# datawhalechina/torch-rechub

Measured on AMD Instinct MI355X. Metric: CTR train samples/sec, DeepFM Criteo-shape synthetic, higher is better.
Workload: dtype f32

## Files before the change

torch_rechub_amd/csrc/optim.hip:

```cpp
#include "common.h"
#include "wgrad_body.h"

namespace {

constexpr int kMaxTensors = 128;
constexpr int kMaxRing = 1024;
int g_sweep_grid = 0;
int g_deferred_grid = 512;
int g_gate_ns = 32000;
int g_stagger_ns = 15000;

constexpr int kVecPerThread = 4;
constexpr int kChunk4 = RH_BLOCK * kVecPerThread;

struct AdamArgs {
  const int64_t* tdesc;
  const double* hyper;
  int T;
  int zero_grad;
  int64_t total_vblocks;
  int64_t vb_prefix[kMaxTensors + 1];
};

__global__ void adam_prepare_kernel(double* hyper, int64_t* step, float* ring, int64_t ring_mask) {
  RH_CHAIN_PRIO();
  if (threadIdx.x == 0 && blockIdx.x == 0) {
    const int64_t t = *step + 1;
    *step = t;
    const double lr = hyper[0], b1 = hyper[1], b2 = hyper[2];
    const double bc1 = 1.0 - pow(b1, (double)t);
    const double bc2 = 1.0 - pow(b2, (double)t);
    hyper[8] = lr / bc1;
    hyper[9] = sqrt(bc2);
    hyper[10] = 1.0 - b1;
    hyper[11] = 1.0 - b2;
    hyper[12] = (double)t;
    const double A = hyper[8] * hyper[9], E = hyper[3] * hyper[9];
    hyper[13] = A;
    hyper[14] = E;
    if (ring != nullptr) {
      ring[2 * (t & ring_mask) + 0] = (float)A;
      ring[2 * (t & ring_mask) + 1] = (float)E;
    }
  }
}

struct AdamScalars {
  float b1, b2, wd, one_m_b1, one_m_b2;
  float c1wd, c2wd2;
  float A, E;
};

static __device__ __forceinline__ void adam_elem(float& p, float g, float& m, float& v, const AdamScalars& h, float A,
                                                 float E) {
  g = fmaf(h.wd, p, g);
  m = fmaf(h.one_m_b1, g - m, m);
  v = fmaf(h.one_m_b2, g * g, v * h.b2);
  p = fmaf(-A, m * __builtin_amdgcn_rcpf(__builtin_amdgcn_sqrtf(v) + E), p);
}
typedef float rh_v2f __attribute__((ext_vector_type(2)));
static __device__ __forceinline__ void adam_pair(rh_v2f& p, rh_v2f g, rh_v2f& m, rh_v2f& v, const AdamScalars& h,
                                                 float A, float E) {
  g = __builtin_elementwise_fma(rh_v2f{h.wd, h.wd}, p, g);
  m = __builtin_elementwise_fma(rh_v2f{h.one_m_b1, h.one_m_b1}, g - m, m);
  v = __builtin_elementwise_fma(rh_v2f{h.one_m_b2, h.one_m_b2}, g * g, v * h.b2);
  rh_v2f d = rh_v2f{__builtin_amdgcn_sqrtf(v.x), __builtin_amdgcn_sqrtf(v.y)} + E;
  d = rh_v2f{__builtin_amdgcn_rcpf(d.x), __builtin_amdgcn_rcpf(d.y)};
  p = __builtin_elementwise_fma(rh_v2f{-A, -A}, m * d, p);
}
static __device__ __forceinline__ void adam_pair_zero_g(rh_v2f& p, rh_v2f& m, rh_v2f& v, const AdamScalars& h, float A,
                                                        float E) {
  m = __builtin_elementwise_fma(rh_v2f{h.c1wd, h.c1wd}, p, m * h.b1);
  v = __builtin_elementwise_fma(rh_v2f{h.c2wd2, h.c2wd2}, p * p, v * h.b2);
  rh_v2f d = rh_v2f{__builtin_amdgcn_sqrtf(v.x), __builtin_amdgcn_sqrtf(v.y)} + E;
  d = rh_v2f{__builtin_amdgcn_rcpf(d.x), __builtin_amdgcn_rcpf(d.y)};
  p = __builtin_elementwise_fma(rh_v2f{-A, -A}, m * d, p);
}
static __device__ __forceinline__ void adam_f4_zero_g(float4& P, float4& M, float4& V, const AdamScalars& h, float A,
                                                      float E) {
  rh_v2f p0{P.x, P.y}, p1{P.z, P.w}, m0{M.x, M.y}, m1{M.z, M.w}, v0{V.x, V.y}, v1{V.z, V.w};
  adam_pair_zero_g(p0, m0, v0, h, A, E);
  adam_pair_zero_g(p1, m1, v1, h, A, E);
  P = make_float4(p0.x, p0.y, p1.x, p1.y);
  M = make_float4(m0.x, m0.y, m1.x, m1.y);
  V = make_float4(v0.x, v0.y, v1.x, v1.y);
}
static __device__ __forceinline__ void adam_f4(float4& P, const float4 G, float4& M, float4& V, const AdamScalars& h,
                                               float A, float E) {
  float4 Pz = P, Mz = M, Vz = V;
  adam_f4_zero_g(Pz, Mz, Vz, h, A, E);
  rh_v2f p0{P.x, P.y}, p1{P.z, P.w}, m0{M.x, M.y}, m1{M.z, M.w}, v0{V.x, V.y}, v1{V.z, V.w};
  adam_pair(p0, rh_v2f{G.x, G.y}, m0, v0, h, A, E);
  adam_pair(p1, rh_v2f{G.z, G.w}, m1, v1, h, A, E);
  P = make_float4(G.x == 0.f ? Pz.x : p0.x, G.y == 0.f ? Pz.y : p0.y, G.z == 0.f ? Pz.z : p1.x, G.w == 0.f ? Pz.w : p1.y);
  M = make_float4(G.x == 0.f ? Mz.x : m0.x, G.y == 0.f ? Mz.y : m0.y, G.z == 0.f ? Mz.z : m1.x, G.w == 0.f ? Mz.w : m1.y);
  V = make_float4(G.x == 0.f ? Vz.x : v0.x, G.y == 0.f ? Vz.y : v0.y, G.z == 0.f ? Vz.z : v1.x, G.w == 0.f ? Vz.w : v1.y);
}
static __device__ __forceinline__ AdamScalars load_scalars(const double* hyper) {
  AdamScalars h;
  h.b1 = (float)hyper[1];
  h.b2 = (float)hyper[2];
  h.wd = (float)hyper[4];
  h.one_m_b1 = (float)hyper[10];
  h.one_m_b2 = (float)hyper[11];
  h.c1wd = h.one_m_b1 * h.wd;
  h.c2wd2 = h.one_m_b2 * h.wd * h.wd;
  h.A = (float)hyper[13];
  h.E = (float)hyper[14];
  return h;
}

__global__ __launch_bounds__(RH_BLOCK) void adam_dense_kernel(const AdamArgs a) {
  const AdamScalars h = load_scalars(a.hyper);
  const int T = a.T;
  for (int64_t vb = blockIdx.x; vb < a.total_vblocks; vb += gridDim.x) {
    int lo = 0, hi = T;
    while (hi - lo > 1) {
      const int mid = (lo + hi) >> 1;
      if (a.vb_prefix[mid] <= vb) lo = mid; else hi = mid;
    }
    const int t = lo;
    float* p = reinterpret_cast<float*>(a.tdesc[0 * T + t]);
    float* g = reinterpret_cast<float*>(a.tdesc[1 * T + t]);
    float* m = reinterpret_cast<float*>(a.tdesc[2 * T + t]);
    float* v = reinterpret_cast<float*>(a.tdesc[3 * T + t]);
    const int64_t n4 = a.tdesc[4 * T + t] / 4;
    const int64_t base4 = (vb - a.vb_prefix[t]) * kChunk4;
    float4 P[kVecPerThread], Gv[kVecPerThread], M[kVecPerThread], V[kVecPerThread];
    bool ok[kVecPerThread];
#pragma unroll
    for (int k = 0; k < kVecPerThread; ++k) {
      const int64_t i4 = base4 + (int64_t)k * RH_BLOCK + threadIdx.x;
      ok[k] = i4 < n4;
      const int64_t j4 = ok[k] ? i4 : 0;
      P[k] = gload<float4>(p + j4 * 4);
      Gv[k] = gload<float4>(g + j4 * 4);
      M[k] = gload<float4>(m + j4 * 4);
      V[k] = gload<float4>(v + j4 * 4);
    }
#pragma unroll
    for (int k = 0; k < kVecPerThread; ++k) {
      if (!ok[k]) continue;
      const int64_t i4 = base4 + (int64_t)k * RH_BLOCK + threadIdx.x;
      const bool gnz = Gv[k].x != 0.f || Gv[k].y != 0.f || Gv[k].z != 0.f || Gv[k].w != 0.f;
      adam_f4(P[k], Gv[k], M[k], V[k], h, h.A, h.E);
      gstore<float4>(p + i4 * 4, P[k]);
      gstore<float4>(m + i4 * 4, M[k]);
      gstore<float4>(v + i4 * 4, V[k]);
      if (a.zero_grad && gnz) gstore<float4>(g + i4 * 4, f4_zero());
    }
  }
}


struct LazyTouchedArgs {
  const int64_t* ldesc;
  const int64_t* field_table;
  const int64_t* idesc;
  const double* hyper;
  const float* ring;
  int ring_mask;
  int T, B, F, spb;
  int* err;
  const int64_t* perm;
  const int64_t* pos;
  int64_t N;
  const int64_t* src_sparse;
  int Fd;
  const float* src_dense;
  int ND;
  const float* src_label;
  int64_t* sparse_out;
  float* dense_out;
  float* label_out;
  int look;
  int look_n;
  int64_t off;
};

struct LazySweepArgs {
  const int64_t* ldesc;
  const double* hyper;
  const float* ring;
  int ring_mask;
  int T;
  int flush;
  int64_t t_value;
  int64_t total_vblocks;
  int64_t vb_prefix[kMaxTensors + 1];
  int touch_blocks, touch_chunks, touch_period;
  int touch_i32;
  LazyTouchedArgs touch;
};

template <int LPR, typename IdxT, bool REFRESH, bool ASSEMBLE = false, bool LOOK = false, bool GRAD = !REFRESH>
static __device__ __forceinline__ void lazy_touched_body(const LazyTouchedArgs& a, int bx, int f);

template <int LPR, bool MERGED>
static __device__ __forceinline__ void lazy_sweep_body(const LazySweepArgs& a, const int bx_, const int gdim_) {
  constexpr int RPB = RH_BLOCK / LPR;
  constexpr int D = 4 * LPR;
  int64_t bid = bx_, nblk = gdim_;
  if (MERGED) {
    const int bx = bx_, P = a.touch_period;
    const int slot_ = bx / P;
    if (bx % P == 0 && slot_ < a.touch_blocks) {
      if (a.touch_i32)
        lazy_touched_body<LPR, int, false>(a.touch, slot_ % a.touch_chunks, slot_ / a.touch_chunks);
      else
        lazy_touched_body<LPR, int64_t, false>(a.touch, slot_ % a.touch_chunks, slot_ / a.touch_chunks);
      return;
    }
    bid = bx - (slot_ + 1 < a.touch_blocks ? slot_ + 1 : a.touch_blocks);
    nblk = (int64_t)gdim_ - a.touch_blocks;
  }
  AdamScalars h = load_scalars(a.hyper);
  const int t = a.t_value >= 0 ? (int)a.t_value : (int)a.hyper[12];
  if (a.t_value >= 0) {
    h.A = a.ring[2 * (t & a.ring_mask)];
    h.E = a.ring[2 * (t & a.ring_mask) + 1];
  }
  const int T = a.T;
  const int q = threadIdx.x % LPR;
  const int slot = threadIdx.x / LPR;
  __shared__ float ring_s[2 * kMaxRing];
  for (int i = threadIdx.x; i < 2 * (a.ring_mask + 1); i += RH_BLOCK) ring_s[i] = a.ring[i];
  __syncthreads();

  struct Unit {
    float *p, *g, *m, *v;
    int* last;
    int64_t r;
    int old;
    bool live, with_g, claimed;
    float4 P, M, V, G;
  };
  auto fetch = [&](int64_t vb, Unit& u) {
    u.live = false;
    if (vb >= a.total_vblocks) return;
    int lo = 0, hi = T;
    while (hi - lo > 1) {
      const int mid = (lo + hi) >> 1;
      if (a.vb_prefix[mid] <= vb) lo = mid; else hi = mid;
    }
    const int ti = lo;
    u.p = reinterpret_cast<float*>(a.ldesc[0 * T + ti]);
    u.g = reinterpret_cast<float*>(a.ldesc[1 * T + ti]);
    u.m = reinterpret_cast<float*>(a.ldesc[2 * T + ti]);
    u.v = reinterpret_cast<float*>(a.ldesc[3 * T + ti]);
    u.last = reinterpret_cast<int*>(a.ldesc[4 * T + ti]);
    const int64_t rows = a.ldesc[5 * T + ti];
    const int64_t K = a.ldesc[6 * T + ti];
    const int64_t w = a.flush ? rows : a.ldesc[7 * T + ti];
    const int64_t wstart = a.flush ? 0 : ((int64_t)(t - 1) % K) * w;
    const int64_t local = (vb - a.vb_prefix[ti]) * RPB + slot;
    u.r = wstart + local;
    if (local >= w || u.r >= rows) return;
    u.with_g = (K == 1);
    const bool claim = MERGED && K != 1;
    u.claimed = claim;
    if (claim) {
      u.old = t;
      if (q == 0) u.old = atomicMax(u.last + u.r, t);
      u.with_g = true;
    } else {
      u.old = gload<int>(u.last + u.r);
    }
    u.P = gload<float4>(u.p + u.r * D + q * 4);
    u.M = gload<float4>(u.m + u.r * D + q * 4);
    u.V = gload<float4>(u.v + u.r * D + q * 4);
    u.G = u.with_g ? gload<float4>(u.g + u.r * D + q * 4) : f4_zero();
    if (claim) u.old = __shfl(u.old, (int)(threadIdx.x % RH_WAVE) - q, RH_WAVE);
    u.live = true;
  };
  auto process = [&](Unit& u) {
    const bool work = u.live && u.old < t;
    const int first = work ? u.old + 1 : t;
    int j = wave_min_uniform(first);
    while (j < t) {
      const int nxt = wave_min_uniform(first > j ? first : t);
      if (first <= j) {
        int jj = j;
        for (; jj + 2 <= nxt; jj += 2) {
          const float2 ae0 = *reinterpret_cast<const float2*>(ring_s + 2 * (jj & a.ring_mask));
          const float2 ae1 = *reinterpret_cast<const float2*>(ring_s + 2 * ((jj + 1) & a.ring_mask));
          __builtin_amdgcn_sched_barrier(0);
          adam_f4_zero_g(u.P, u.M, u.V, h, ae0.x, ae0.y);
          adam_f4_zero_g(u.P, u.M, u.V, h, ae1.x, ae1.y);
        }
        if (jj < nxt) {
          const float2 ae = *reinterpret_cast<const float2*>(ring_s + 2 * (jj & a.ring_mask));
          adam_f4_zero_g(u.P, u.M, u.V, h, ae.x, ae.y);
        }
      }
      j = nxt;
    }
    if (work) {
      if (u.with_g) adam_f4(u.P, u.G, u.M, u.V, h, h.A, h.E);
      else adam_f4_zero_g(u.P, u.M, u.V, h, h.A, h.E);
      gstore<float4>(u.p + u.r * D + q * 4, u.P);
      gstore<float4>(u.m + u.r * D + q * 4, u.M);
      gstore<float4>(u.v + u.r * D + q * 4, u.V);
      if (u.with_g && (u.G.x != 0.f || u.G.y != 0.f || u.G.z != 0.f || u.G.w != 0.f))
        gstore<float4>(u.g + u.r * D + q * 4, f4_zero());
      if (q == 0 && !(MERGED && u.with_g && u.claimed)) u.last[u.r] = t;
    }
  };
  Unit ua, ub;
  fetch(bid, ua);
  for (int64_t vb = bid; vb < a.total_vblocks; vb += 2 * nblk) {
    fetch(vb + nblk, ub);
    process(ua);
    fetch(vb + 2 * nblk, ua);
    process(ub);
  }
}

template <int LPR, bool MERGED = false>
__global__ __launch_bounds__(RH_BLOCK) void adam_lazy_sweep_kernel(const LazySweepArgs a) {
  lazy_sweep_body<LPR, MERGED>(a, (int)blockIdx.x, (int)gridDim.x);
}

template <int LPR, int VPL>
static __device__ __forceinline__ void lazy_sweep_wide_body(const LazySweepArgs& a, const int bx_, const int gdim_) {
  constexpr int RPB = RH_BLOCK / LPR;
  constexpr int D = 4 * LPR * VPL;
  const int64_t bid = bx_, nblk = gdim_;
  AdamScalars h = load_scalars(a.hyper);
  const int t = (int)a.t_value;
  h.A = a.ring[2 * (t & a.ring_mask)];
  h.E = a.ring[2 * (t & a.ring_mask) + 1];
  const int T = a.T;
  const int q = threadIdx.x % LPR;
  const int slot = threadIdx.x / LPR;
  __shared__ float ring_s[2 * kMaxRing];
  for (int i = threadIdx.x; i < 2 * (a.ring_mask + 1); i += RH_BLOCK) ring_s[i] = a.ring[i];
  __syncthreads();
  struct Unit {
    float *p, *m, *v;
    int* last;
    int64_t off;
    int64_t r;
    int old;
    bool live;
    float4 P[VPL], M[VPL], V[VPL];
  };
  auto fetch = [&](int64_t vb, Unit& u) {
    u.live = false;
    if (vb >= a.total_vblocks) return;
    int lo = 0, hi = T;
    while (hi - lo > 1) {
      const int mid = (lo + hi) >> 1;
      if (a.vb_prefix[mid] <= vb) lo = mid; else hi = mid;
    }
    const int ti = lo;
    u.p = reinterpret_cast<float*>(a.ldesc[0 * T + ti]);
    u.m = reinterpret_cast<float*>(a.ldesc[2 * T + ti]);
    u.v = reinterpret_cast<float*>(a.ldesc[3 * T + ti]);
    u.last = reinterpret_cast<int*>(a.ldesc[4 * T + ti]);
    const int64_t rows = a.ldesc[5 * T + ti];
    const int64_t K = a.ldesc[6 * T + ti];
    const int64_t w = a.ldesc[7 * T + ti];
    const int64_t wstart = ((int64_t)(t - 1) % K) * w;
    const int64_t local = (vb - a.vb_prefix[ti]) * RPB + slot;
    u.r = wstart + local;
    if (local >= w || u.r >= rows) return;
    u.off = u.r * D + (int64_t)q * (4 * VPL);
    u.old = gload<int>(u.last + u.r);
#pragma unroll
    for (int k = 0; k < VPL; ++k) {
      u.P[k] = gload<float4>(u.p + u.off + 4 * k);
      u.M[k] = gload<float4>(u.m + u.off + 4 * k);
      u.V[k] = gload<float4>(u.v + u.off + 4 * k);
    }
    u.live = true;
  };
  auto process = [&](Unit& u) {
    const bool work = u.live && u.old < t;
    const int first = work ? u.old + 1 : t;
    int j = wave_min_uniform(first);
    while (j < t) {
      const int nxt = wave_min_uniform(first > j ? first : t);
      if (first <= j) {
        int jj = j;
        for (; jj + 2 <= nxt; jj += 2) {
          const float2 ae0 = *reinterpret_cast<const float2*>(ring_s + 2 * (jj & a.ring_mask));
          const float2 ae1 = *reinterpret_cast<const float2*>(ring_s + 2 * ((jj + 1) & a.ring_mask));
          __builtin_amdgcn_sched_barrier(0);
#pragma unroll
          for (int k = 0; k < VPL; ++k) adam_f4_zero_g(u.P[k], u.M[k], u.V[k], h, ae0.x, ae0.y);
#pragma unroll
          for (int k = 0; k < VPL; ++k) adam_f4_zero_g(u.P[k], u.M[k], u.V[k], h, ae1.x, ae1.y);
        }
        if (jj < nxt) {
          const float2 ae = *reinterpret_cast<const float2*>(ring_s + 2 * (jj & a.ring_mask));
#pragma unroll
          for (int k = 0; k < VPL; ++k) adam_f4_zero_g(u.P[k], u.M[k], u.V[k], h, ae.x, ae.y);
        }
      }
      j = nxt;
    }
    if (work) {
#pragma unroll
      for (int k = 0; k < VPL; ++k) {
        adam_f4_zero_g(u.P[k], u.M[k], u.V[k], h, h.A, h.E);
        gstore<float4>(u.p + u.off + 4 * k, u.P[k]);
        gstore<float4>(u.m + u.off + 4 * k, u.M[k]);
        gstore<float4>(u.v + u.off + 4 * k, u.V[k]);
      }
      if (q == 0) u.last[u.r] = t;
    }
  };
  Unit ua, ub;
  fetch(bid, ua);
  for (int64_t vb = bid; vb < a.total_vblocks; vb += 2 * nblk) {
    fetch(vb + nblk, ub);
    process(ua);
    fetch(vb + 2 * nblk, ua);
    process(ub);
  }
}

template <int LPR, int VPL>
__global__ __launch_bounds__(RH_BLOCK) void adam_lazy_sweep_wide_kernel(const LazySweepArgs a) {
  lazy_sweep_wide_body<LPR, VPL>(a, (int)blockIdx.x, (int)gridDim.x);
}

__global__ void stream_delay_kernel(const long long ticks) {
  const long long t0 = wall_clock64();
  while (wall_clock64() - t0 < ticks) __builtin_amdgcn_s_sleep(16);
}

__global__ void stream_gate_kernel(const long long* gate, const long long expected, const long long ticks, const long long timeout,
                                   int* err, long long* done_host, const long long done_value) {
  if (done_host != nullptr) __hip_atomic_store(done_host, done_value, __ATOMIC_RELAXED, __HIP_MEMORY_SCOPE_SYSTEM);
  const long long t0 = wall_clock64();
  while (__hip_atomic_load(gate, __ATOMIC_ACQUIRE, __HIP_MEMORY_SCOPE_AGENT) - expected < 0) {
    __builtin_amdgcn_s_sleep(8);
    if (wall_clock64() - t0 > timeout) {
      if (err != nullptr) atomicOr(err, RH_ERR_GATE_TIMEOUT);
      return;
    }
  }
  const int slot = 4 + 2 * (int)(expected & 3);
  const long long base = __hip_atomic_load(gate + slot, __ATOMIC_RELAXED, __HIP_MEMORY_SCOPE_AGENT);
  const long long opened = __hip_atomic_load(gate + slot + 1, __ATOMIC_RELAXED, __HIP_MEMORY_SCOPE_AGENT);
  while (__hip_atomic_load(gate + 2, __ATOMIC_RELAXED, __HIP_MEMORY_SCOPE_AGENT) - base < 1 && wall_clock64() - opened < ticks)
    __builtin_amdgcn_s_sleep(4);
}

static __device__ __forceinline__ void gate_open(long long* gate) {
  const long long idx = __hip_atomic_load(gate, __ATOMIC_RELAXED, __HIP_MEMORY_SCOPE_AGENT) + 1;
  const int slot = 4 + 2 * (int)(idx & 3);
  const long long now = (long long)wall_clock64();
  __hip_atomic_store(gate + slot, __hip_atomic_load(gate + 2, __ATOMIC_RELAXED, __HIP_MEMORY_SCOPE_AGENT), __ATOMIC_RELAXED,
                     __HIP_MEMORY_SCOPE_AGENT);
  __hip_atomic_store(gate + slot + 1, now, __ATOMIC_RELAXED, __HIP_MEMORY_SCOPE_AGENT);
  __hip_atomic_store(gate + 1, now, __ATOMIC_RELAXED, __HIP_MEMORY_SCOPE_AGENT);
  __hip_atomic_fetch_add(gate, 1ll, __ATOMIC_RELEASE, __HIP_MEMORY_SCOPE_AGENT);
}

__global__ void stream_gate_open_kernel(long long* gate) { gate_open(gate); }
__global__ void stream_gate_release_kernel(long long* gate) {
  __hip_atomic_fetch_add(gate + 2, 1ll, __ATOMIC_RELAXED, __HIP_MEMORY_SCOPE_AGENT);
}

template <int LPR, typename IdxT, bool REFRESH, bool ASSEMBLE, bool LOOK, bool GRAD>
static __device__ __forceinline__ void lazy_touched_body(const LazyTouchedArgs& a, int bx, int f) {
  constexpr int LPP = RH_BLOCK / LPR;
  constexpr int D = 4 * LPR;
  const int T = a.T, F = a.F;
  const int64_t ti = a.field_table[f];
  if (ti < 0) return;
  const int64_t K = a.ldesc[6 * T + ti];
  if (K == 1) return;
  const int64_t pad = a.field_table[F + f];
  float* p = reinterpret_cast<float*>(a.ldesc[0 * T + ti]);
  float* g = reinterpret_cast<float*>(a.ldesc[1 * T + ti]);
  float* m = reinterpret_cast<float*>(a.ldesc[2 * T + ti]);
  float* v = reinterpret_cast<float*>(a.ldesc[3 * T + ti]);
  int* last = reinterpret_cast<int*>(a.ldesc[4 * T + ti]);
  const int64_t rows = a.ldesc[5 * T + ti];
  const IdxT* ip = reinterpret_cast<const IdxT*>(a.idesc[f]);
  const int64_t st = a.idesc[F + f];
  const int64_t acol = ASSEMBLE ? (reinterpret_cast<const int64_t*>(ip) - a.sparse_out) : 0;
  const int64_t apos = ASSEMBLE ? a.pos[0] : 0;
  const AdamScalars h = load_scalars(a.hyper);
  const int t = (int)a.hyper[12];
  const int q = threadIdx.x % LPR;
  const int slot = threadIdx.x / LPR;
  const int lane = threadIdx.x % RH_WAVE;
  const int64_t nsamp = LOOK ? a.look_n : a.B;
  int64_t b0 = (int64_t)bx * (LOOK ? a.look : a.spb);
  int64_t b1 = (b0 + (LOOK ? a.look : a.spb) < nsamp) ? b0 + (LOOK ? a.look : a.spb) : nsamp;
  __shared__ float ring_t[REFRESH ? 2 * kMaxRing : 2];
  if (REFRESH) {
    for (int i = threadIdx.x; i < 2 * (a.ring_mask + 1); i += RH_BLOCK) ring_t[i] = a.ring[i];
    __syncthreads();
  }
  const float* ring = REFRESH ? ring_t : a.ring;
  const bool pad_pass = !LOOK && REFRESH && pad >= 0 && pad < rows && bx == 0;
  __shared__ int64_t s_look[LOOK ? RH_BLOCK : 1];
  __shared__ int s_nlook;
  const int64_t look_b1 = b1;
  for (int64_t sub = LOOK ? b0 : 0; sub < (LOOK ? look_b1 : 1); sub += RH_BLOCK) {
  if (LOOK) {
    const int64_t w = a.ldesc[7 * T + ti];
    const int64_t ws = ((int64_t)(t - 1) % K) * w;
    if (threadIdx.x == 0) s_nlook = 0;
    __syncthreads();
    const int64_t b = sub + threadIdx.x;
    if (b < look_b1) {
      const int64_t p = (apos + a.off + (int64_t)a.B + b) % a.N;
      const int64_t r = gload<int64_t>(a.src_sparse + gload<int64_t>(a.perm + p) * a.Fd + acol);
      if (r >= ws && r < ws + w && r < rows && r != pad) s_look[atomicAdd(&s_nlook, 1)] = r;
    }
    __syncthreads();
    b0 = 0;
    b1 = s_nlook;
  }
  const int64_t b_end = b1 + (pad_pass ? LPP : 0);
  for (int64_t base = b0; base < b_end; base += LPP) {
    const bool extra = base >= b1;
    const int64_t b = base + slot;
    const bool ok = !extra && b < b1;
    int64_t r;
    if (LOOK) {
      r = s_look[ok ? b : 0];
    } else if (ASSEMBLE) {
      int64_t p = apos + a.off + (ok ? b : b1 - 1);
      if (p >= a.N) p %= a.N;
      if (p < 0) p += a.N;
      r = gload<int64_t>(a.src_sparse + gload<int64_t>(a.perm + p) * a.Fd + acol);
    } else {
      r = (int64_t)gload<IdxT>(ip + (ok ? b : b1 - 1) * st);
    }
    bool valid = ok && (uint64_t)r < (uint64_t)rows && r != pad;
    if (extra) {
      r = pad;
      valid = slot == 0;
    }
    int old = t;
    if (valid && q == 0) {
      old = gload<int>(last + r);
      if (old < t) old = atomicMax(last + r, t);
    }
    old = __shfl(old, lane - q, RH_WAVE);
    bool act = valid && old < t;
    int64_t rr = r;
    if (REFRESH) {
      __shared__ int s_key[LPP];
      __shared__ int s_old[LPP];
      __shared__ int64_t s_row[LPP];
      const int lag = act ? t - old : 0;
      __syncthreads();
      if (q == 0) s_key[slot] = lag;
      __syncthreads();
      int rank = 0;
#pragma unroll 4
      for (int j = 0; j < LPP; ++j) {
        const int kj = s_key[j];
        rank += (kj > lag || (kj == lag && j < slot)) ? 1 : 0;
      }
      constexpr int kPerWave = RH_WAVE / LPR;
      rank = (rank + (bx % (LPP / kPerWave > 0 ? LPP / kPerWave : 1)) * kPerWave) % LPP;
      if (q == 0) {
        s_row[rank] = r;
        s_old[rank] = act ? old : t;
      }
      __syncthreads();
      rr = s_row[slot];
      old = s_old[slot];
      act = old < t;
    }
    float4 P = f4_zero(), M = f4_zero(), V = f4_zero(), G = f4_zero();
    if (act) {
      P = gload<float4>(p + rr * D + q * 4);
      M = gload<float4>(m + rr * D + q * 4);
      V = gload<float4>(v + rr * D + q * 4);
      if (GRAD) G = gload<float4>(g + rr * D + q * 4);
    }
    const int first = act ? old + 1 : t;
    int j = wave_min_uniform(first);
    while (j < t) {
      const int nxt = wave_min_uniform(first > j ? first : t);
      if (first <= j) {
        for (int jj = j; jj < nxt; ++jj) {
          const float A = ring[2 * (jj & a.ring_mask)], E = ring[2 * (jj & a.ring_mask) + 1];
          adam_f4_zero_g(P, M, V, h, A, E);
        }
      }
      j = nxt;
    }
    if (!act) continue;
    if (GRAD) adam_f4(P, G, M, V, h, h.A, h.E);
    else adam_f4_zero_g(P, M, V, h, h.A, h.E);
    gstore<float4>(p + rr * D + q * 4, P);
    gstore<float4>(m + rr * D + q * 4, M);
    gstore<float4>(v + rr * D + q * 4, V);
    if (GRAD && (!REFRESH || G.x != 0.f || G.y != 0.f || G.z != 0.f || G.w != 0.f)) gstore<float4>(g + rr * D + q * 4, f4_zero());
  }
  }
}

template <int LPR, typename IdxT, bool REFRESH>
__global__ __launch_bounds__(RH_BLOCK) void adam_lazy_touched_kernel(const LazyTouchedArgs a) {
  RH_CHAIN_PRIO();
  lazy_touched_body<LPR, IdxT, REFRESH>(a, (int)blockIdx.x, (int)blockIdx.y);
}

constexpr int kTouchGroup = 4;
struct LazyTouchedGroupArgs {
  LazyTouchedArgs rec[kTouchGroup];
  int prefix[kTouchGroup + 1];
  int chunks[kTouchGroup];
  int i64[kTouchGroup];
  int n;
};

template <int LPR, bool REFRESH>
__global__ __launch_bounds__(RH_BLOCK) void adam_lazy_touched_group_kernel(const LazyTouchedGroupArgs g) {
  RH_CHAIN_PRIO();
  const int bx = (int)blockIdx.x;
  int i = 0;
#pragma unroll
  for (int k = 1; k < kTouchGroup; ++k) i += (k < g.n && bx >= g.prefix[k]) ? 1 : 0;
  const int local = bx - g.prefix[i];
#pragma unroll
  for (int k = 0; k < kTouchGroup; ++k) {
    if (k == i) {
      if (g.i64[k]) lazy_touched_body<LPR, int64_t, REFRESH>(g.rec[k], local % g.chunks[k], local / g.chunks[k]);
      else lazy_touched_body<LPR, int, REFRESH>(g.rec[k], local % g.chunks[k], local / g.chunks[k]);
      return;
    }
  }
}

template <int LPR>
__global__ __launch_bounds__(RH_BLOCK) void adam_lazy_refresh_assemble_kernel(const LazyTouchedArgs a) {
  RH_CHAIN_PRIO();
  if ((int)blockIdx.y < a.F) {
    lazy_touched_body<LPR, int64_t, true, true>(a, (int)blockIdx.x, (int)blockIdx.y);
    return;
  }
  if ((int)blockIdx.y > a.F) {
    const int R = a.look / a.spb;
    const int f = ((int)blockIdx.y - a.F - 1) * R + (int)blockIdx.x % R;
    if (f < a.F) lazy_touched_body<LPR, int64_t, true, true, true>(a, (int)blockIdx.x / R, f);
    return;
  }
  constexpr int G = 16;
  const int lig = threadIdx.x % G;
  const int64_t pos = a.pos[0];
  const int64_t b0 = (int64_t)blockIdx.x * a.spb;
  const int64_t b1 = (b0 + a.spb < (int64_t)a.B) ? b0 + a.spb : (int64_t)a.B;
  for (int64_t b = b0 + threadIdx.x / G; b < b1; b += RH_BLOCK / G) {
    int64_t p = pos + b;
    if (p >= a.N) p %= a.N;
    const int64_t src = a.perm[p];
    for (int j = lig; j < a.Fd; j += G) a.sparse_out[b * a.Fd + j] = a.src_sparse[src * a.Fd + j];
    for (int j = lig; j < a.ND; j += G) a.dense_out[b * a.ND + j] = a.src_dense[src * a.ND + j];
    if (lig == 0 && a.src_label != nullptr) a.label_out[b] = a.src_label[src];
  }
}

struct StepAheadParts {
  int nB, chunksB;
  int spbB;
  int nA, chunksA;
  int spbA;
  int nC, chunksC;
  int nD;
  const int64_t* idescA;
  int BA;
};

template <int LPR>
__device__ __forceinline__ void step_ahead_body(const LazySweepArgs& a, const StepAheadParts& parts, int bx, const int nblocks) {
  if (bx < parts.nB) {
    LazyTouchedArgs ta = a.touch;
    ta.spb = parts.spbB;
    ta.off = 0;
    lazy_touched_body<LPR, int64_t, true, true, false, true>(ta, bx % parts.chunksB, bx / parts.chunksB);
    return;
  }
  bx -= parts.nB;
  if (bx < parts.nA) {
    LazyTouchedArgs ta = a.touch;
    ta.spb = parts.spbA;
    if (parts.BA > 0) {
      ta.idesc = parts.idescA;
      ta.B = parts.BA;
      ta.off = 0;
      lazy_touched_body<LPR, int64_t, false, false, false, true>(ta, bx % parts.chunksA, bx / parts.chunksA);
      return;
    }
    ta.off = -(int64_t)ta.B;
    lazy_touched_body<LPR, int64_t, false, true, false, true>(ta, bx % parts.chunksA, bx / parts.chunksA);
    return;
  }
  bx -= parts.nA;
  if (bx < parts.nC) {
    LazyTouchedArgs ta = a.touch;
    ta.off = 0;
    lazy_touched_body<LPR, int64_t, true, true, true, true>(ta, bx % parts.chunksC, bx / parts.chunksC);
    return;
  }
  bx -= parts.nC;
  if (bx < parts.nD) {
    const LazyTouchedArgs& ta = a.touch;
    constexpr int G = 16;
    const int lig = threadIdx.x % G;
    const int64_t pos = ta.pos[0];
    const int64_t b0 = (int64_t)bx * parts.spbB;
    const int64_t b1 = (b0 + parts.spbB < (int64_t)ta.B) ? b0 + parts.spbB : (int64_t)ta.B;
    for (int64_t b = b0 + threadIdx.x / G; b < b1; b += RH_BLOCK / G) {
      int64_t p = pos + b;
      if (p >= ta.N) p %= ta.N;
      const int64_t src = ta.perm[p];
      for (int j = lig; j < ta.Fd; j += G) ta.sparse_out[b * ta.Fd + j] = ta.src_sparse[src * ta.Fd + j];
      for (int j = lig; j < ta.ND; j += G) ta.dense_out[b * ta.ND + j] = ta.src_dense[src * ta.ND + j];
      if (lig == 0 && ta.src_label != nullptr) ta.label_out[b] = ta.src_label[src];
    }
    return;
  }
  bx -= parts.nD;
  lazy_sweep_body<LPR, true>(a, bx, nblocks - parts.nB - parts.nA - parts.nC - parts.nD);
}

template <int LPR>
__global__ __launch_bounds__(RH_BLOCK) void adam_lazy_step_ahead_kernel(const LazySweepArgs a, const StepAheadParts parts) {
  RH_CHAIN_PRIO();
  step_ahead_body<LPR>(a, parts, (int)blockIdx.x, (int)gridDim.x);
}

template <int LPR>
__global__ __launch_bounds__(RH_BLOCK) __attribute__((amdgpu_waves_per_eu(4, 4))) void adam_lazy_step_ahead_wgrad_kernel(
    const LazySweepArgs a, const StepAheadParts parts, const rh_wgrad::WgradGroupArgs ga) {
  RH_CHAIN_PRIO();
  extern __shared__ float wred[];
  const int nW = ga.prefix[rh_wgrad::kWgradGroup];
  const int nrest = (int)gridDim.x - nW;
  const int bx = (int)blockIdx.x;
  if (bx >= nrest) {
    rh_wgrad::linear_wgrad_group_body<true>(ga, wred, bx - nrest);
    return;
  }
  step_ahead_body<LPR>(a, parts, bx, nrest);
}

template <int LPR, int VPL>
int launch_sweep_wide(LazySweepArgs& a, const int64_t* h_rows, const int64_t* h_window, hipStream_t s) {
  constexpr int RPB = RH_BLOCK / LPR;
  a.vb_prefix[0] = 0;
  for (int t = 0; t < a.T; ++t) {
    int64_t w = h_window[t] < h_rows[t] ? h_window[t] : h_rows[t];
    if (h_window[t] >= h_rows[t]) w = 0;
    a.vb_prefix[t + 1] = a.vb_prefix[t] + (w + RPB - 1) / RPB;
  }
  for (int t = a.T + 1; t <= kMaxTensors; ++t) a.vb_prefix[t] = a.vb_prefix[a.T];
  a.total_vblocks = a.vb_prefix[a.T];
  a.touch_blocks = a.touch_chunks = 0;
  a.touch_period = 1;
  if (a.total_vblocks == 0) return 0;
  int64_t grid = a.total_vblocks;
  const int64_t cap = g_deferred_grid > 0 ? g_deferred_grid : (g_sweep_grid > 0 ? g_sweep_grid : 256 * 32);
  if (grid > cap) grid = cap;
  hipLaunchKernelGGL((adam_lazy_sweep_wide_kernel<LPR, VPL>), dim3((unsigned)grid), dim3(RH_BLOCK), 0, s, a);
  return 0;
}

template <int LPR>
int launch_sweep(LazySweepArgs& a, int mode, const int64_t* h_rows, const int64_t* h_window, hipStream_t s,
                 const LazyTouchedArgs* touch = nullptr) {
  constexpr int RPB = RH_BLOCK / LPR;
  if constexpr (LPR >= 2) {
    if (mode == RH_SWEEP_LAZY_TABLES && a.t_value >= 0 && touch == nullptr)
      return launch_sweep_wide<LPR / 2, 2>(a, h_rows, h_window, s);
  }
  a.vb_prefix[0] = 0;
  for (int t = 0; t < a.T; ++t) {
    int64_t w = a.flush ? h_rows[t] : (h_window[t] < h_rows[t] ? h_window[t] : h_rows[t]);
    const bool dense_table = h_window[t] >= h_rows[t];
    if ((mode == RH_SWEEP_LAZY_TABLES && dense_table) || (mode == RH_SWEEP_DENSE_TABLES && !dense_table)) w = 0;
    a.vb_prefix[t + 1] = a.vb_prefix[t] + (w + RPB - 1) / RPB;
  }
  for (int t = a.T + 1; t <= kMaxTensors; ++t) a.vb_prefix[t] = a.vb_prefix[a.T];
  a.total_vblocks = a.vb_prefix[a.T];
  a.touch_blocks = a.touch_chunks = 0;
  a.touch_period = 1;
  if (touch != nullptr) {
    a.touch = *touch;
    a.touch_chunks = (touch->B + touch->spb - 1) / touch->spb;
    a.touch_blocks = a.touch_chunks * touch->F;
  }
  if (a.total_vblocks == 0 && a.touch_blocks == 0) return 0;
  int64_t grid = a.total_vblocks;
  const int64_t cap = (a.t_value >= 0 && touch == nullptr && g_deferred_grid > 0) ? g_deferred_grid
                      : (g_sweep_grid > 0 ? g_sweep_grid : 256 * 32);
  if (grid > cap) grid = cap;
  if (touch != nullptr) {
    if (grid < 1) grid = 1;
    int64_t period = (grid + a.touch_blocks) / a.touch_blocks;
    if (period > 1 && period % 8 == 0) period -= 1;
    a.touch_period = (int)period;
    hipLaunchKernelGGL((adam_lazy_sweep_kernel<LPR, true>), dim3((unsigned)(grid + a.touch_blocks)), dim3(RH_BLOCK), 0, s,
                       a);
  } else {
    hipLaunchKernelGGL((adam_lazy_sweep_kernel<LPR, false>), dim3((unsigned)grid), dim3(RH_BLOCK), 0, s, a);
  }
  return 0;
}


struct AdamSmallArgs {
  const int64_t* sdesc;
  const float* flat_g;
  const double* hyper;
  int T;
  int64_t total_vblocks;
  int64_t vb_prefix[kMaxTensors + 1];
};
constexpr int kSmallChunk = 1024;

__global__ __launch_bounds__(RH_BLOCK) void adam_small_kernel(const AdamSmallArgs a) {
  RH_CHAIN_PRIO();
  const AdamScalars h = load_scalars(a.hyper);
  const int T = a.T;
  for (int64_t vb = blockIdx.x; vb < a.total_vblocks; vb += gridDim.x) {
    int lo = 0, hi = T;
    while (hi - lo > 1) {
      const int mid = (lo + hi) >> 1;
      if (a.vb_prefix[mid] <= vb) lo = mid; else hi = mid;
    }
    const int t = lo;
    float* p = reinterpret_cast<float*>(a.sdesc[0 * T + t]);
    float* m = reinterpret_cast<float*>(a.sdesc[1 * T + t]);
    float* v = reinterpret_cast<float*>(a.sdesc[2 * T + t]);
    const int64_t n = a.sdesc[3 * T + t];
    const float* g = a.flat_g + a.sdesc[4 * T + t];
    const int64_t base = (vb - a.vb_prefix[t]) * kSmallChunk;
#pragma unroll
    for (int k = 0; k < kSmallChunk / RH_BLOCK; ++k) {
      const int64_t i = base + (int64_t)k * RH_BLOCK + threadIdx.x;
      if (i < n) {
        float P = p[i], M = m[i], V = v[i];
        adam_elem(P, g[i], M, V, h, h.A, h.E);
        p[i] = P;
        m[i] = M;
        v[i] = V;
      }
    }
  }
}

constexpr int kPackItems = 32;
struct PackArgs {
  RhPackItem it[kPackItems];
  int64_t vb_prefix[kPackItems + 1];
  int n;
  float* flat;
  const int64_t* sdesc;
  const double* hyper;
  int T, base;
  long long* gate;
};

static __device__ __forceinline__ void pack_adam(const PackArgs& a, const AdamScalars& h, int item, int64_t i, float g) {
  const int t = a.base + item;
  float* p = reinterpret_cast<float*>(a.sdesc[0 * a.T + t]);
  float* m = reinterpret_cast<float*>(a.sdesc[1 * a.T + t]);
  float* v = reinterpret_cast<float*>(a.sdesc[2 * a.T + t]);
  float P = p[i], M = m[i], V = v[i];
  adam_elem(P, g, M, V, h, h.A, h.E);
  p[i] = P;
  m[i] = M;
  v[i] = V;
}
constexpr int kPackChunk = RH_BLOCK;
constexpr int kPackDeep = 32;

template <bool ADAM>
static __device__ __forceinline__ void pack_body(const PackArgs& a, const int bx_, const int gdim_) {
  __shared__ float red[RH_BLOCK / RH_WAVE];
  AdamScalars h{};
  if (ADAM) h = load_scalars(a.hyper);
  for (int64_t vb = bx_; vb < a.vb_prefix[a.n]; vb += gdim_) {
    int lo = 0, hi = a.n;
    while (hi - lo > 1) {
      const int mid = (lo + hi) >> 1;
      if (a.vb_prefix[mid] <= vb) lo = mid; else hi = mid;
    }
    const RhPackItem& it = a.it[lo];
    const float* src = reinterpret_cast<const float*>(it.src);
    const float* add = reinterpret_cast<const float*>(it.add);
    float* dst = a.flat + it.dst_offset;
    if (it.numel < 64 && it.nparts > 64) {
      __syncthreads();
      for (int64_t e = 0; e < it.numel; ++e) {
        float acc = 0.f;
        for (int64_t r = threadIdx.x; r < it.nparts; r += RH_BLOCK) acc += src[r * it.stride + e];
        acc = wave_sum(acc);
        if (threadIdx.x % RH_WAVE == 0) red[threadIdx.x / RH_WAVE] = acc;
        __syncthreads();
        if (threadIdx.x == 0) {
          const float gsum = (((red[0] + red[1]) + red[2]) + red[3]) + (add ? add[e] : 0.f);
          dst[e] = gsum;
          if (ADAM) pack_adam(a, h, lo, e, gsum);
        }
        __syncthreads();
      }
      continue;
    }
    if (it.nparts > kPackDeep) {
      const int wave = threadIdx.x / RH_WAVE, lane = threadIdx.x % RH_WAVE;
      const int64_t i = (vb - a.vb_prefix[lo]) * RH_WAVE + lane;
      float v = 0.f;
      if (i < it.numel) {
        int64_t r = wave;
        for (; r + 28 < it.nparts; r += 32) {
          float t[8];
#pragma unroll
          for (int k = 0; k < 8; ++k) t[k] = src[(r + 4 * k) * it.stride + i];
#pragma unroll
          for (int k = 0; k < 8; ++k) v += t[k];
        }
        for (; r < it.nparts; r += 4) v += src[r * it.stride + i];
      }
      __shared__ float deep[RH_BLOCK];
      __syncthreads();
      deep[threadIdx.x] = v;
      __syncthreads();
      if (wave == 0 && i < it.numel) {
        const float gsum = (((deep[lane] + deep[RH_WAVE + lane]) + deep[2 * RH_WAVE + lane]) + deep[3 * RH_WAVE + lane]) +
                           (add ? add[i] : 0.f);
        dst[i] = gsum;
        if (ADAM) pack_adam(a, h, lo, i, gsum);
      }
      continue;
    }
    const int64_t i = (vb - a.vb_prefix[lo]) * kPackChunk + threadIdx.x;
    if (i < it.numel) {
      float v = 0.f;
      int64_t r = 0;
      for (; r + 4 <= it.nparts; r += 4) {
        const float t0 = src[(r + 0) * it.stride + i], t1 = src[(r + 1) * it.stride + i];
        const float t2 = src[(r + 2) * it.stride + i], t3 = src[(r + 3) * it.stride + i];
        v = (((v + t0) + t1) + t2) + t3;
      }
      for (; r < it.nparts; ++r) v += src[r * it.stride + i];
      if (add) v += add[i];
      dst[i] = v;
      if (ADAM) pack_adam(a, h, lo, i, v);
    }
  }
}

template <bool ADAM>
__global__ __launch_bounds__(RH_BLOCK) void pack_grads_kernel(const PackArgs a) {
  RH_CHAIN_PRIO();
  if (a.gate != nullptr && blockIdx.x == 0 && threadIdx.x == 0) gate_open(a.gate);
  pack_body<ADAM>(a, (int)blockIdx.x, (int)gridDim.x);
}

static bool pack_fill(PackArgs& a, const RhPackItem* items, int base) {
  a.vb_prefix[0] = 0;
  for (int i = 0; i < a.n; ++i) {
    const RhPackItem& it = items[base + i];
    if (!(it.numel >= 0 && it.nparts >= 0 && it.dst_offset >= 0 && (it.nparts == 0 || it.src != 0))) return false;
    a.it[i] = it;
    const bool tall = it.numel < 64 && it.nparts > 64;
    const int64_t per = it.nparts > kPackDeep ? RH_WAVE : kPackChunk;
    a.vb_prefix[i + 1] = a.vb_prefix[i] + (tall ? 1 : (it.numel + per - 1) / per);
  }
  for (int i = a.n; i < kPackItems; ++i) a.vb_prefix[i + 1] = a.vb_prefix[a.n];
  return true;
}

}

static int pack_impl(const RhPackItem* items, int n, float* flat, const int64_t* sdesc, const double* hyper, void* stream,
                     int64_t* gate = nullptr) {
  RH_REQUIRE(items != nullptr && flat != nullptr && n >= 0, RH_E_BADARG, "rh_pack_grads: null pointer");
  hipStream_t st = reinterpret_cast<hipStream_t>(stream);
  for (int base = 0; base < n; base += kPackItems) {
    PackArgs a;
    a.n = n - base < kPackItems ? n - base : kPackItems;
    a.flat = flat;
    a.sdesc = sdesc;
    a.hyper = hyper;
    a.T = n;
    a.base = base;
    a.gate = base == 0 ? reinterpret_cast<long long*>(gate) : nullptr;
    RH_REQUIRE(pack_fill(a, items, base), RH_E_BADARG, "rh_pack_grads: bad item in [%d, %d)", base, base + a.n);
    if (a.vb_prefix[a.n] == 0) continue;
    int64_t grid = a.vb_prefix[a.n];
    if (grid > 4096) grid = 4096;
    if (sdesc != nullptr) hipLaunchKernelGGL(pack_grads_kernel<true>, dim3((unsigned)grid), dim3(RH_BLOCK), 0, st, a);
    else hipLaunchKernelGGL(pack_grads_kernel<false>, dim3((unsigned)grid), dim3(RH_BLOCK), 0, st, a);
  }
  RH_LAUNCH_CHECK("rh_pack_grads");
  return 0;
}

extern "C" int rh_pack_grads(const RhPackItem* items, int n, float* flat, void* stream) {
  return pack_impl(items, n, flat, nullptr, nullptr, stream);
}

extern "C" int rh_pack_grads_adam(const RhPackItem* items, int n, float* flat, const int64_t* sdesc, const double* hyper,
                                  void* stream) {
  RH_REQUIRE(sdesc != nullptr && hyper != nullptr, RH_E_BADARG, "rh_pack_grads_adam: null pointer");
  return pack_impl(items, n, flat, sdesc, hyper, stream);
}

extern "C" int rh_pack_grads_adam_gate(const RhPackItem* items, int n, float* flat, const int64_t* sdesc, const double* hyper,
                                       int64_t* gate, void* stream) {
  RH_REQUIRE(sdesc != nullptr && hyper != nullptr && n >= 1, RH_E_BADARG, "rh_pack_grads_adam_gate: null pointer");
  return pack_impl(items, n, flat, sdesc, hyper, stream, gate);
}

extern "C" int rh_optim_set_tuning(int key, int value) {
  if (key == RH_TUNE_SWEEP_GRID) {
    g_sweep_grid = value;
    return 0;
  }
  if (key == RH_TUNE_DEFERRED_GRID) {
    g_deferred_grid = value;
    return 0;
  }
  if (key == RH_TUNE_SWEEP_STAGGER_NS) {
    g_stagger_ns = value;
    return 0;
  }
  if (key == RH_TUNE_SWEEP_GATE_NS) {
    g_gate_ns = value;
    return 0;
  }
  return RH_E_BADARG;
}

extern "C" int rh_adam_prepare(double* hyper, int64_t* step, float* ring, int ring_size, void* stream) {
  RH_REQUIRE(hyper != nullptr && step != nullptr, RH_E_BADARG, "rh_adam_prepare: null pointer");
  RH_REQUIRE(ring == nullptr || (ring_size > 0 && (ring_size & (ring_size - 1)) == 0), RH_E_BADARG,
             "rh_adam_prepare: ring_size must be a power of two");
  hipLaunchKernelGGL(adam_prepare_kernel, dim3(1), dim3(64), 0, reinterpret_cast<hipStream_t>(stream), hyper,
                     step, ring, (int64_t)(ring_size - 1));
  RH_LAUNCH_CHECK("rh_adam_prepare");
  return 0;
}

extern "C" int rh_adam_dense(const int64_t* tdesc, int T, const int64_t* h_numel, const double* hyper,
                             int zero_grad, void* stream) {
  RH_REQUIRE(tdesc != nullptr && h_numel != nullptr && hyper != nullptr, RH_E_BADARG,
             "rh_adam_dense: null pointer");
  RH_REQUIRE(T >= 1 && T <= kMaxTensors, RH_E_UNSUPPORTED, "rh_adam_dense: T=%d (max %d tensors per call)", T,
             kMaxTensors);
  AdamArgs a;
  a.tdesc = tdesc;
  a.hyper = hyper;
  a.T = T;
  a.zero_grad = zero_grad;
  a.vb_prefix[0] = 0;
  for (int t = 0; t < T; ++t) {
    RH_REQUIRE(h_numel[t] >= 0 && h_numel[t] % 4 == 0, RH_E_BADARG,
               "rh_adam_dense: numel[%d]=%lld must be a non-negative multiple of 4", t, (long long)h_numel[t]);
    const int64_t n4 = h_numel[t] / 4;
    a.vb_prefix[t + 1] = a.vb_prefix[t] + (n4 + kChunk4 - 1) / kChunk4;
  }
  for (int t = T + 1; t <= kMaxTensors; ++t) a.vb_prefix[t] = a.vb_prefix[T];
  a.total_vblocks = a.vb_prefix[T];
// ... 444 lines not shown
```

Before: 18.65 million.

## Split lazy Adam sweep into replay/store phases and spread wide-sweep tail blocks

The lazy Adam sweep kernels now separate the replay computation from the stores, with an explicit waitcnt/sched barrier between them, so memory operations are ordered and overlapped more predictably. The wide sweep also rebalances the ragged final round: leftover vblocks beyond a whole multiple of the grid are split into narrow single-vector sub-passes and handed to strided blocks before their main loop. This avoids a few blocks running a lone extra iteration at the end. Descriptor loads are moved to the constant address space. These changes add template complexity, and the strict waitcnt may stall the wave more often.

```diff
diff --git a/torch_rechub_amd/csrc/optim.hip b/torch_rechub_amd/csrc/optim.hip
--- a/torch_rechub_amd/csrc/optim.hip
+++ b/torch_rechub_amd/csrc/optim.hip
@@ -1,3 +1,5 @@
+#include <type_traits>
+
 #include "common.h"
 #include "wgrad_body.h"
 
@@ -187,6 +189,8 @@
   int flush;
   int64_t t_value;
   int64_t total_vblocks;
+  int64_t walk_vblocks;
+  int tail_passes, tail_stride;
   int64_t vb_prefix[kMaxTensors + 1];
   int touch_blocks, touch_chunks, touch_period;
   int touch_i32;
@@ -273,7 +277,12 @@
     if (claim) u.old = __shfl(u.old, (int)(threadIdx.x % RH_WAVE) - q, RH_WAVE);
     u.live = true;
   };
-  auto process = [&](Unit& u) {
+  auto settle = [&]() {
+    __builtin_amdgcn_sched_barrier(0);
+    __builtin_amdgcn_s_waitcnt(0x0F70);
+    __builtin_amdgcn_sched_barrier(0);
+  };
+  auto replay = [&](Unit& u) {
     const bool work = u.live && u.old < t;
     const int first = work ? u.old + 1 : t;
     int j = wave_min_uniform(first);
@@ -298,6 +307,10 @@
     if (work) {
       if (u.with_g) adam_f4(u.P, u.G, u.M, u.V, h, h.A, h.E);
       else adam_f4_zero_g(u.P, u.M, u.V, h, h.A, h.E);
+    }
+  };
+  auto store = [&](Unit& u) {
+    if (u.live && u.old < t) {
       gstore<float4>(u.p + u.r * D + q * 4, u.P);
       gstore<float4>(u.m + u.r * D + q * 4, u.M);
       gstore<float4>(u.v + u.r * D + q * 4, u.V);
@@ -308,11 +321,16 @@
   };
   Unit ua, ub;
   fetch(bid, ua);
+  settle();
   for (int64_t vb = bid; vb < a.total_vblocks; vb += 2 * nblk) {
     fetch(vb + nblk, ub);
-    process(ua);
+    replay(ua);
+    settle();
+    store(ua);
     fetch(vb + 2 * nblk, ua);
-    process(ub);
+    replay(ub);
+    settle();
+    store(ub);
   }
 }
 
@@ -320,6 +338,18 @@
 __global__ __launch_bounds__(RH_BLOCK) void adam_lazy_sweep_kernel(const LazySweepArgs a) {
   lazy_sweep_body<LPR, MERGED>(a, (int)blockIdx.x, (int)gridDim.x);
 }
+
+template <int NV>
+struct WideSweepUnit {
+  static constexpr int kNV = NV;
+  float *p, *m, *v;
+  int* last;
+  int64_t off;
+  int64_t r;
+  int old;
+  bool live;
+  float4 P[NV], M[NV], V[NV];
+};
 
 template <int LPR, int VPL>
 static __device__ __forceinline__ void lazy_sweep_wide_body(const LazySweepArgs& a, const int bx_, const int gdim_) {
@@ -331,51 +361,52 @@
   h.A = a.ring[2 * (t & a.ring_mask)];
   h.E = a.ring[2 * (t & a.ring_mask) + 1];
   const int T = a.T;
-  const int q = threadIdx.x % LPR;
-  const int slot = threadIdx.x / LPR;
   __shared__ float ring_s[2 * kMaxRing];
   for (int i = threadIdx.x; i < 2 * (a.ring_mask + 1); i += RH_BLOCK) ring_s[i] = a.ring[i];
   __syncthreads();
-  struct Unit {
-    float *p, *m, *v;
-    int* last;
-    int64_t off;
-    int64_t r;
-    int old;
-    bool live;
-    float4 P[VPL], M[VPL], V[VPL];
-  };
-  auto fetch = [&](int64_t vb, Unit& u) {
+  using Wide = WideSweepUnit<VPL>;
+  using Narrow = WideSweepUnit<1>;
+  auto fetch = [&](auto& u, int64_t vb, int sub, int64_t end) {
+    constexpr int NV = std::remove_reference_t<decltype(u)>::kNV;
+    constexpr int LPRU = D / (4 * NV);
     u.live = false;
-    if (vb >= a.total_vblocks) return;
+    if (vb >= end) return;
     int lo = 0, hi = T;
     while (hi - lo > 1) {
       const int mid = (lo + hi) >> 1;
       if (a.vb_prefix[mid] <= vb) lo = mid; else hi = mid;
     }
     const int ti = lo;
-    u.p = reinterpret_cast<float*>(a.ldesc[0 * T + ti]);
-    u.m = reinterpret_cast<float*>(a.ldesc[2 * T + ti]);
-    u.v = reinterpret_cast<float*>(a.ldesc[3 * T + ti]);
-    u.last = reinterpret_cast<int*>(a.ldesc[4 * T + ti]);
-    const int64_t rows = a.ldesc[5 * T + ti];
-    const int64_t K = a.ldesc[6 * T + ti];
-    const int64_t w = a.ldesc[7 * T + ti];
+    typedef __attribute__((address_space(4))) const int64_t* kdesc_t;
+    kdesc_t ld = (kdesc_t)a.ldesc;
+    u.p = reinterpret_cast<float*>(ld[0 * T + ti]);
+    u.m = reinterpret_cast<float*>(ld[2 * T + ti]);
+    u.v = reinterpret_cast<float*>(ld[3 * T + ti]);
+    u.last = reinterpret_cast<int*>(ld[4 * T + ti]);
+    const int64_t rows = ld[5 * T + ti];
+    const int64_t K = ld[6 * T + ti];
+    const int64_t w = ld[7 * T + ti];
     const int64_t wstart = ((int64_t)(t - 1) % K) * w;
-    const int64_t local = (vb - a.vb_prefix[ti]) * RPB + slot;
+    const int64_t local = (vb - a.vb_prefix[ti]) * RPB + sub * (RH_BLOCK / LPRU) + (int)threadIdx.x / LPRU;
     u.r = wstart + local;
     if (local >= w || u.r >= rows) return;
-    u.off = u.r * D + (int64_t)q * (4 * VPL);
+    u.off = u.r * D + (int64_t)((int)threadIdx.x % LPRU) * (4 * NV);
     u.old = gload<int>(u.last + u.r);
 #pragma unroll
-    for (int k = 0; k < VPL; ++k) {
+    for (int k = 0; k < NV; ++k) {
       u.P[k] = gload<float4>(u.p + u.off + 4 * k);
       u.M[k] = gload<float4>(u.m + u.off + 4 * k);
       u.V[k] = gload<float4>(u.v + u.off + 4 * k);
     }
     u.live = true;
   };
-  auto process = [&](Unit& u) {
+  auto settle = [&]() {
+    __builtin_amdgcn_sched_barrier(0);
+    __builtin_amdgcn_s_waitcnt(0x0F70);
+    __builtin_amdgcn_sched_barrier(0);
+  };
+  auto replay = [&](auto& u) {
+    constexpr int NV = std::remove_reference_t<decltype(u)>::kNV;
     const bool work = u.live && u.old < t;
     const int first = work ? u.old + 1 : t;
     int j = wave_min_uniform(first);
@@ -388,36 +419,59 @@
           const float2 ae1 = *reinterpret_cast<const float2*>(ring_s + 2 * ((jj + 1) & a.ring_mask));
           __builtin_amdgcn_sched_barrier(0);
 #pragma unroll
-          for (int k = 0; k < VPL; ++k) adam_f4_zero_g(u.P[k], u.M[k], u.V[k], h, ae0.x, ae0.y);
+          for (int k = 0; k < NV; ++k) adam_f4_zero_g(u.P[k], u.M[k], u.V[k], h, ae0.x, ae0.y);
 #pragma unroll
-          for (int k = 0; k < VPL; ++k) adam_f4_zero_g(u.P[k], u.M[k], u.V[k], h, ae1.x, ae1.y);
+          for (int k = 0; k < NV; ++k) adam_f4_zero_g(u.P[k], u.M[k], u.V[k], h, ae1.x, ae1.y);
         }
         if (jj < nxt) {
           const float2 ae = *reinterpret_cast<const float2*>(ring_s + 2 * (jj & a.ring_mask));
 #pragma unroll
-          for (int k = 0; k < VPL; ++k) adam_f4_zero_g(u.P[k], u.M[k], u.V[k], h, ae.x, ae.y);
+          for (int k = 0; k < NV; ++k) adam_f4_zero_g(u.P[k], u.M[k], u.V[k], h, ae.x, ae.y);
         }
       }
       j = nxt;
     }
     if (work) {
 #pragma unroll
-      for (int k = 0; k < VPL; ++k) {
-        adam_f4_zero_g(u.P[k], u.M[k], u.V[k], h, h.A, h.E);
+      for (int k = 0; k < NV; ++k) adam_f4_zero_g(u.P[k], u.M[k], u.V[k], h, h.A, h.E);
+    }
+  };
+  auto store = [&](auto& u) {
+    constexpr int NV = std::remove_reference_t<decltype(u)>::kNV;
+    constexpr int LPRU = D / (4 * NV);
+    if (u.live && u.old < t) {
+#pragma unroll
+      for (int k = 0; k < NV; ++k) {
         gstore<float4>(u.p + u.off + 4 * k, u.P[k]);
         gstore<float4>(u.m + u.off + 4 * k, u.M[k]);
         gstore<float4>(u.v + u.off + 4 * k, u.V[k]);
       }
-      if (q == 0) u.last[u.r] = t;
+      if ((int)threadIdx.x % LPRU == 0) u.last[u.r] = t;
     }
   };
-  Unit ua, ub;
-  fetch(bid, ua);
-  for (int64_t vb = bid; vb < a.total_vblocks; vb += 2 * nblk) {
-    fetch(vb + nblk, ub);
-    process(ua);
-    fetch(vb + 2 * nblk, ua);
-    process(ub);
+  Wide ua, ub;
+  if (a.tail_passes > 0 && bid % a.tail_stride == 0 && bid / a.tail_stride < a.tail_passes) {
+    const int64_t pass = bid / a.tail_stride;
+    Narrow un;
+    fetch(un, a.walk_vblocks + pass / VPL, (int)(pass % VPL), a.total_vblocks);
+    settle();
+    fetch(ua, bid, 0, a.walk_vblocks);
+    replay(un);
+    settle();
+    store(un);
+  } else {
+    fetch(ua, bid, 0, a.walk_vblocks);
+    settle();
+  }
+  for (int64_t vb = bid; vb < a.walk_vblocks; vb += 2 * nblk) {
+    fetch(ub, vb + nblk, 0, a.walk_vblocks);
+    replay(ua);
+    settle();
+    store(ua);
+    fetch(ua, vb + 2 * nblk, 0, a.walk_vblocks);
+    replay(ub);
+    settle();
+    store(ub);
   }
 }
 
@@ -766,6 +820,15 @@
   int64_t grid = a.total_vblocks;
   const int64_t cap = g_deferred_grid > 0 ? g_deferred_grid : (g_sweep_grid > 0 ? g_sweep_grid : 256 * 32);
   if (grid > cap) grid = cap;
+  const int64_t R = a.total_vblocks / grid, rem = a.total_vblocks - R * grid;
+  a.walk_vblocks = a.total_vblocks;
+  a.tail_passes = 0;
+  a.tail_stride = 1;
+  if (R >= 1 && rem > 0 && rem <= grid / 4) {
+    a.walk_vblocks = R * grid;
+    a.tail_passes = (int)(rem * VPL);
+    a.tail_stride = (int)(grid / a.tail_passes);
+  }
   hipLaunchKernelGGL((adam_lazy_sweep_wide_kernel<LPR, VPL>), dim3((unsigned)grid), dim3(RH_BLOCK), 0, s, a);
   return 0;
 }
```

New measurement: 18.55 million. No clear change (-0.5%).
